# PCCproject/PCC-RL

Measured on AMD Instinct MI355X. Metric: env steps/sec (whole node) at 64k parallel envs, higher is better.
Workload: dtype f64; 1 GPU; BASELINE config 3: 65536 envs/GPU, 1 sender, per-env randomized bw/latency/queue/loss (ICML'19 ranges), U(-1,1) actions, 400-step episodes, auto-reset; envs_per_gpu=65536, senders=1, episode_return_allgathers=0, step_launches=two (send_kernel, retire_kernel)

## Files before the change

pcc-rl_amd/csrc/pcc_dev.h:

```cpp
#pragma once
#include <hip/hip_runtime.h>
#include <cstddef>

#include <cmath>
#include <cstdarg>
#include <cstdint>
#include <cstdio>
#include <cstdlib>
#include <cstring>
#include <atomic>
#include <new>
#include <vector>

#include "pcc_sim.h"

namespace pcc {

constexpr int kMaxFeatures = 16;
constexpr int kMaxSenders = 2;
constexpr int kWave = 64;
constexpr int kRetireBlock = 128;
#ifndef PCC_RETIRE_OCC
#define PCC_RETIRE_OCC 4
#endif
// ... 35 lines not shown
    uint32_t ha, hd, ta, td;
    uint32_t mi_sent;
    uint32_t ring_held[kMaxTiers];
    uint32_t cwnd;
    uint32_t heap_n;
    uint32_t send_cost;
    float ack_rate, loss_rate;
    uint32_t on_return_a, on_return_d;
};
static_assert(sizeof(EnvBlk) == 128 && sizeof(SndBlk) == 128, "one line per block");

struct NoiseOut {
    double now, q, tu, nsend;
    uint32_t sent, acked, lost, flags;
    uint32_t seq, pad[3];
};
static_assert(sizeof(NoiseOut) == 64, "one 64-byte record per env");

struct Dev {
    int64_t n;
    int ns, H, F, HF;
    int32_t fid[kMaxFeatures];
    int n_tiers;
    uint32_t cap0;
    char *tier_base[kMaxTiers];
    uint32_t *pool_free;
    size_t pool_free_stride;
    uint32_t *pool_share;
    int32_t *tier_top;
    uint32_t tier_slots[kMaxTiers];
    uint32_t parts, parts_shift, part_envs;
    uint32_t key0, key1, gid_base;
    uint32_t params_gen;
    double delta_scale;
    uint32_t max_steps;
    uint32_t *cls_count;
    uint32_t *cls_list;
    uint32_t *cursors;
    uint32_t *fctl;
    unsigned long long *q_entries;
    uint32_t q_cap;
    uint32_t fused_acquire;
    uint32_t fused_spin_ticks;
    uint32_t fused_debug;
    uint32_t fused_partial_naps;
    uint32_t fused_max_naps;
    uint32_t *any_done;
    uint32_t step_seq;
    uint64_t *timeline;
    unsigned long long *pass_stats;
    int pass_counters;
    uint32_t light_snake, wave_oldest_first, prio_level, prio_light_items, prio_wave_items, prio_team;
    uint32_t retire_sorted;
    int debug_skip;
    uint32_t round_packets, takeover_lanes, send_envs_per_wave, send_waves;
    double heavy_predict;
    double team_predict;
    float heavy_item_packets;
    float light_half_predict;
    float retire_wide_predict;
    double lo[5], hi[5];
    int rng_mode;
    const double *trace;
    int64_t trace_stride;
    const double *p_bw, *p_dl, *p_queue, *p_loss, *p_rate0;
    EnvBlk *env;
    SndBlk *snd;
    int64_t stride;
    char *shadow_rings;
    uint32_t *refill_count;
    uint32_t *refill_list;
    int shadows;
    unsigned long long *restart_stats;
    int use_cwnd;
    int use_noise;
    int engine;
    double noise_span;
    uint32_t noise_cap;
    double2 *noise_heap;
    double2 *noise_rtt;
    NoiseOut *noise_out;
    uint32_t noise_seq;
    float *hist;
    double2 *ring;
};

}
using namespace pcc;

namespace {

#ifndef PCC_PROFILE
#define PCC_PROFILE 0
#endif
constexpr bool kProfile = PCC_PROFILE != 0;
__device__ __forceinline__ bool prof_on(const Dev &D) { return kProfile && D.timeline != nullptr; }
__device__ __forceinline__ bool prof_counters(const Dev &D) { return kProfile && D.pass_counters != 0; }
__device__ __forceinline__ bool prof_skip(const Dev &D, int bit) { return kProfile && (D.debug_skip & bit) != 0; }

__device__ __forceinline__ double max0(double x) { return x > 0.0 ? x : 0.0; }

__device__ __forceinline__ void set_prio(uint32_t level) {
    if (level == 1u) __builtin_amdgcn_s_setprio(1);
    else if (level == 2u) __builtin_amdgcn_s_setprio(2);
    else if (level >= 3u) __builtin_amdgcn_s_setprio(3);
    else __builtin_amdgcn_s_setprio(0);
}

__device__ __forceinline__ uint64_t mul_wide_u32(uint32_t a, uint32_t b) {
    uint64_t r;
    asm("v_mad_u64_u32 %0, vcc, %1, %2, 0" : "=v"(r) : "v"(a), "v"(b) : "vcc");
    return r;
}

__device__ __forceinline__ void philox4x32_10(uint32_t c0, uint32_t c1, uint32_t c2, uint32_t c3, uint32_t k0,
                                              uint32_t k1, uint32_t (&out)[4]) {
#pragma unroll
    for (int r = 0; r < 10; r++) {
        const uint64_t p0 = mul_wide_u32(c0, 0xD2511F53u), p1 = mul_wide_u32(c2, 0xCD9E8D57u);
        const uint32_t hi0 = (uint32_t)(p0 >> 32), lo0 = (uint32_t)p0;
        const uint32_t hi1 = (uint32_t)(p1 >> 32), lo1 = (uint32_t)p1;
        const uint32_t n0 = hi1 ^ c1 ^ k0, n2 = hi0 ^ c3 ^ k1;
        c0 = n0; c1 = lo1; c2 = n2; c3 = lo0;
        k0 += 0x9E3779B9u; k1 += 0xBB67AE85u;
    }
    out[0] = c0; out[1] = c1; out[2] = c2; out[3] = c3;
}

__device__ __forceinline__ void philox4x32_10_sched(uint32_t c0, uint32_t c1, uint32_t c2, uint32_t c3, uint32_t k0,
                                                    uint32_t k1, uint32_t (&out)[4]) {
#pragma unroll
    for (int r = 0; r < 10; r++) {
        const uint64_t p0 = (uint64_t)c0 * 0xD2511F53u, p1 = (uint64_t)c2 * 0xCD9E8D57u;
        const uint32_t hi0 = (uint32_t)(p0 >> 32), lo0 = (uint32_t)p0;
        const uint32_t hi1 = (uint32_t)(p1 >> 32), lo1 = (uint32_t)p1;
        const uint32_t n0 = hi1 ^ c1 ^ k0, n2 = hi0 ^ c3 ^ k1;
        c0 = n0; c1 = lo1; c2 = n2; c3 = lo0;
        k0 += 0x9E3779B9u; k1 += 0xBB67AE85u;
    }
    out[0] = c0; out[1] = c1; out[2] = c2; out[3] = c3;
}

__device__ __forceinline__ double u32_to_unit(uint32_t x) { return (double)x * (1.0 / 4294967296.0); }

__device__ __forceinline__ double philox_packet_uniform(const Dev &D, uint32_t gid, uint32_t episode, uint32_t mi,
                                                        uint32_t j) {
    uint32_t w[4];
    philox4x32_10(j >> 2, mi, episode, gid, D.key0, D.key1, w);
    const uint32_t i = j & 3u;
    return u32_to_unit(i == 0 ? w[0] : i == 1 ? w[1] : i == 2 ? w[2] : w[3]);
}

__device__ __forceinline__ double2 link_send(double t, bool rnd , double dl,
                                             double maxq, double ebw, double &q, double &tu, bool &dropped) {
    const double qcur = max0(q - (t - tu));
    const double lat0 = dl + qcur;
    const bool full = ebw + qcur > maxq;
    const double grown = qcur + ebw;
    q = rnd ? q : (full ? qcur : grown);
    tu = rnd ? tu : t;
    dropped = rnd || full;
    double2 rec;
    rec.x = t + lat0;
    rec.y = lat0;
    return rec;
}

constexpr double kNearTol = 1e-12;
// ... 247 lines not shown
```

pcc-rl_amd/csrc/pcc_retire.hip:

```cpp
#include "pcc_retire_env.h"
#include "pcc_kernels.h"

#ifndef PCC_RETIRE_OCC2
#define PCC_RETIRE_OCC2 3
#endif

namespace {

constexpr int kRetireMaxPerBlock = kRetireBlock / 8;

__device__ __forceinline__ float *pol_lds() {
    extern __shared__ float s_pol_dyn[];
    return s_pol_dyn;
}

__device__ __forceinline__ const PolicyArgs &pol_arg(const PolicyArgs &p) { return p; }

template <int NS, bool NOISE, typename... Pol>
__global__ __launch_bounds__(kRetireBlock, NS == 2 ? PCC_RETIRE_OCC2 : PCC_RETIRE_OCC) void retire_kernel(Dev D, int read_buf, int fill_buf, int warm,
                                                              uint32_t warm_mi, int last_warm, int gate, int restart, float *obs_out,
                                                              float *reward_out, uint8_t *done_out, double *steps_out,
                                                              const void *actions, int actions_f64, Pol... pol) {
    constexpr bool POLICY = sizeof...(Pol) > 0;
    if (gate && __hip_atomic_load(D.any_done, __ATOMIC_RELAXED, __HIP_MEMORY_SCOPE_AGENT) != D.step_seq) return;
    __shared__ uint32_t s_env[kRetireMaxPerBlock], s_cls[kRetireMaxPerBlock], s_arrived;
    const uint32_t tid = threadIdx.x;
    if (prof_on(D) && !warm) {
        for (int64_t slot = (int64_t)blockIdx.x * kRetireBlock + tid; slot < 2 * D.n; slot += (int64_t)gridDim.x * kRetireBlock)
            D.timeline[slot * 8] = 0;
    }
    if (prof_on(D) && !warm && blockIdx.x < 8u && tid == 0 && D.n >= 1024)
        D.timeline[(int64_t)19 * D.n + 24 + blockIdx.x] = ((uint64_t)D.step_seq << 8) | xcc_id();
    const uint32_t lane = tid & (kWave - 1);
    if (tid == 0) s_arrived = 0u;
    if (tid < (uint32_t)kRetireMaxPerBlock) s_env[tid] = 0xFFFFFFFFu;
    if constexpr (POLICY) {
        float *w = pol_lds() + kRetireMaxPerBlock * kPolScratch;
        for (int k = (int)tid; k < pol_arg(pol...).n_params; k += kRetireBlock) w[k] = pol_arg(pol...).params[k];
    }
    __syncthreads();
    int64_t i = D.n;
    bool wide = false;
    const uint32_t P = D.parts, part = blockIdx.x % P, b_loc = blockIdx.x / P, grid_loc = gridDim.x / P;
    if (read_buf >= 0) {
        const uint32_t view = list_view(D, read_buf, part);
        const uint32_t row_mine = lane < (uint32_t)kClasses ? (uint32_t)(kClasses - 1) - lane : (uint32_t)kRestart;
        const uint32_t n_mine = lane <= (uint32_t)kClasses ? *cls_count_of(D, view, row_mine) : 0u;
        uint32_t incl = n_mine;
        for (int o = 1; o <= kClasses; o <<= 1) {
            const uint32_t up = (uint32_t)__shfl_up((int)incl, o);
            if (lane >= (uint32_t)o) incl += up;
        }
        const uint32_t total = rl_u32(incl, kClasses);
        const int cls_wide = NOISE ? kClasses : (D.retire_wide_predict >= 1e9f ? kClasses : class_of(D.retire_wide_predict));
        uint32_t n_top = cls_wide < kClasses ? rl_u32(incl, (uint32_t)(kClasses - 1 - cls_wide)) : 0u;
        {
            const uint32_t narrow_all = (total + 15u) / 16u;
            const uint32_t spare = grid_loc > narrow_all + 1u ? grid_loc - narrow_all - 1u : 0u;
            if (n_top > 16u * spare) n_top = 16u * spare;
        }
        const uint32_t wg_wide = (n_top + 7u) / 8u;
        wide = b_loc < wg_wide;
        uint32_t p;
        bool has;
        if (wide) {
            p = b_loc * 8u + tid / 16u;
            has = p < n_top;
        } else {
            p = n_top + (b_loc - wg_wide) * 16u + tid / 8u;
            has = p < total;
        }
        uint32_t lo_l = 0, hi_l = (uint32_t)kClasses;
        for (int it = 0; it < 6; it++) {
            const uint32_t mid = (lo_l + hi_l) >> 1;
            const uint32_t v = (uint32_t)__shfl((int)incl, (int)mid);
            if (lo_l < hi_l) { if (v > p) hi_l = mid; else lo_l = mid + 1u; }
        }
        const uint32_t L = lo_l;
        const uint32_t inc_L = (uint32_t)__shfl((int)incl, (int)L), n_L = (uint32_t)__shfl((int)n_mine, (int)L);
        if (has) {
            const uint32_t row = L < (uint32_t)kClasses ? (uint32_t)(kClasses - 1) - L : (uint32_t)kRestart;
            const uint32_t off = p - (inc_L - n_L);
            i = (int64_t)cls_list_of(D, view, row)[off];
        }
    } else {
        i = (int64_t)blockIdx.x * kRetireMaxPerBlock + tid / 8u;
    }
    float pred = -1.0f;
    Group g;
    uint32_t slot;
    bool glead;
    if (wide) {
        g.lane = tid & 15u;
        g.shift = lane & ~15u;
        slot = tid / 16u;
        glead = g.lane == 0;
        if (i < D.n) {
            pred = retire_env<NS, NOISE, 16>(D, i, g, warm, warm_mi, last_warm, restart, obs_out, reward_out, done_out, steps_out,
                                             actions, actions_f64);
            if constexpr (POLICY)
                policy_group<16>(pol_arg(pol...), pol_lds() + kRetireMaxPerBlock * kPolScratch, pol_lds() + slot * kPolScratch, obs_out + i * D.HF,
                                 i, D.n, g.lane, pol_arg(pol...).t0 + 1);
        }
    } else {
        g.lane = tid & 7u;
        g.shift = lane & ~7u;
        slot = tid / 8u;
        glead = g.lane == 0;
        if (i < D.n) {
            pred = retire_env<NS, NOISE, 8>(D, i, g, warm, warm_mi, last_warm, restart, obs_out, reward_out, done_out, steps_out,
                                            actions, actions_f64);
            if constexpr (POLICY)
                policy_group<8>(pol_arg(pol...), pol_lds() + kRetireMaxPerBlock * kPolScratch, pol_lds() + slot * kPolScratch, obs_out + i * D.HF,
                                i, D.n, g.lane, pol_arg(pol...).t0 + 1);
        }
    }
    if (fill_buf < 0) return;
    if (glead) {
        const bool restarted = pred == -2.0f;
        s_env[slot] = (pred != -1.0f) ? (uint32_t)i : 0xFFFFFFFFu;
        s_cls[slot] = restarted ? (uint32_t)kRestart : (uint32_t)class_of(pred);
    }
    __threadfence_block();
    uint32_t before = 0u;
    if (lane == 0) before = atomicAdd(&s_arrived, 1u);
    before = (uint32_t)__builtin_amdgcn_readfirstlane((int)before);
    if (before != kRetireBlock / kWave - 1) return;
    constexpr int kPerBlock = kRetireMaxPerBlock;
    const uint32_t e = lane < (uint32_t)kPerBlock ? s_env[lane & (kPerBlock - 1)] : 0xFFFFFFFFu;
    const uint32_t c = lane < (uint32_t)kPerBlock ? s_cls[lane & (kPerBlock - 1)] : 0xFFFFFFFFu;
// ... 42 lines not shown
```

pcc-rl_amd/csrc/pcc_retire_env.h:

```cpp
#pragma once
#include "pcc_dev.h"

namespace {

struct Group {
    uint32_t lane;
    uint32_t shift;
};

template <int G>
__device__ __forceinline__ uint32_t gballot(const Group &g, bool p) {
    return (uint32_t)(__ballot(p) >> g.shift) & ((1u << G) - 1u);
}

template <int G>
__device__ __forceinline__ double gbcast(double v, uint32_t src) { return __shfl(v, (int)src, G); }
template <int G>
__device__ __forceinline__ uint32_t gbcast(uint32_t v, uint32_t src) { return (uint32_t)__shfl((int)v, (int)src, G); }
template <int G>
__device__ __forceinline__ uint32_t gbcast(const Group &g, uint32_t v, uint32_t src) {
    return (uint32_t)__builtin_amdgcn_ds_bpermute((int)((g.shift + (src & (uint32_t)(G - 1))) << 2), (int)v);
}
template <int G>
__device__ __forceinline__ double gbcast(const Group &g, double v, uint32_t src) {
    const int idx = (int)((g.shift + (src & (uint32_t)(G - 1))) << 2);
    const int lo = __builtin_amdgcn_ds_bpermute(idx, __double2loint(v)), hi = __builtin_amdgcn_ds_bpermute(idx, __double2hiint(v));
    return __hiloint2double(hi, lo);
}

template <int G>
__device__ __forceinline__ uint32_t search_boundary(const Group &g, const double2 *ring, uint32_t mask, uint32_t lo,
                                                    uint32_t hi, double add, double end) {
    while (hi - lo > (uint32_t)G) {
        const uint32_t stride = (hi - lo + G - 1) / G;
        uint32_t sidx = lo + (g.lane + 1) * stride;
        if (sidx > hi) sidx = hi;
        sidx -= 1;
        const bool pass = ld_t1(ring + (sidx & mask)) + add < end;
        const uint32_t mfail = ~gballot<G>(g, pass) & ((1u << G) - 1u);
        if (!mfail) return hi;
        const uint32_t f = (uint32_t)__ffs((int)mfail) - 1u;
        const uint32_t s_f = gbcast<G>(g, sidx, f);
        if (f) lo = gbcast<G>(g, sidx, f - 1) + 1;
        hi = s_f;
        if (hi < lo) hi = lo;
    }
    const uint32_t k = lo + g.lane;
    const bool fail = k < hi && !(ld_t1(ring + (k & mask)) + add < end);
    const uint32_t m = gballot<G>(g, fail);
    return m ? lo + (uint32_t)__ffs((int)m) - 1u : hi;
}

struct Bound {
    uint32_t b;
    bool clean;
    double t, lat;
};

template <int K, int G>
__device__ __forceinline__ void search_many(const Group &g, const double2 *const (&ring)[K], const uint32_t (&mask)[K],
                                            const uint32_t (&lo0)[K], const uint32_t (&hi0)[K], const double (&add)[K],
                                            double end, const uint32_t (&hint)[K], Bound (&out)[K],
                                            unsigned long long *stat = nullptr ) {
    static_assert(K == 4 && (G == 16 || G == 8), "four searches per group of 16 or 8 lanes");
    constexpr int R = 16 / G;
    uint32_t lo[K], hi[K];
    bool inside[K], below[K];
    bool all_inside = true;
    auto window = [&](const bool (&need)[K], const bool last) {
        double2 r[K][R];
        uint32_t base[K];
#pragma unroll
        for (int k = 0; k < K; k++) {
            base[k] = lo[k] - lo0[k] >= 2u ? lo[k] - 2u : lo0[k];
#pragma unroll
            for (int h = 0; h < R; h++) {
                const uint32_t idx = base[k] + (uint32_t)(h * G) + g.lane;
                r[k][h].x = 0.0; r[k][h].y = 0.0;
                if (need[k] && idx < hi0[k]) r[k][h] = ld_rec(ring[k] + (idx & mask[k]));
            }
        }
#pragma unroll
        for (int k = 0; k < K; k++) {
            if (!need[k]) continue;
            uint32_t mpass = 0, m = 0, mnear = 0;
#pragma unroll
            for (int h = 0; h < R; h++) {
                const uint32_t idx = base[k] + (uint32_t)(h * G) + g.lane;
                const bool in = idx < hi0[k];
                const bool passes = in && (r[k][h].x + add[k] < end);
                mpass |= gballot<G>(g, passes) << (h * G);
                m |= gballot<G>(g, in && idx >= lo[k] && idx < hi[k] && !passes) << (h * G);
                double tn = gbcast<G>(g, r[k][h].x, (g.lane + 1u) & (uint32_t)(G - 1));
                if (h + 1 < R) {
                    const double tw = gbcast<G>(g, r[k][h + 1 < R ? h + 1 : h].x, 0u);
                    if (g.lane == (uint32_t)G - 1u) tn = tw;
                }
                const bool has_next = (h + 1 < R) || g.lane + 1 < (uint32_t)G;
                const bool nr = in && (idx + 1 < hi0[k]) && has_next && near_time(r[k][h].x, tn);
                mnear |= gballot<G>(g, nr) << (h * G);
            }
            const uint32_t b = m ? base[k] + (uint32_t)__ffs((int)m) - 1u : hi[k];
            const bool lo_ok = lo[k] == lo0[k] || ((mpass >> (lo[k] - 1u - base[k])) & 1u);
            const bool hi_ok = hi[k] == hi0[k] || !((mpass >> (hi[k] - base[k])) & 1u);
            inside[k] = last || (lo_ok && hi_ok);
            below[k] = !lo_ok;
            if (!inside[k]) {
                if (!lo_ok) { hi[k] = lo[k] - 1u; lo[k] = lo0[k]; }
                else { lo[k] = hi[k] + 1u; hi[k] = hi0[k]; }
                continue;
            }
            uint32_t want = 0;
            for (int d = 0; d < 3; d++) {
                const int l = (int)(b - base[k]) - 2 + d;
                if (l >= 0 && l < 16) want |= 1u << l;
            }
            out[k].b = b;
            out[k].clean = (mnear & want) == 0u;
            const uint32_t lb = b - base[k] < 16u ? b - base[k] : 0u;
            double bx = r[k][0].x, by = r[k][0].y;
            if (R > 1 && lb >= (uint32_t)G) { bx = r[k][R - 1].x; by = r[k][R - 1].y; }
            out[k].t = gbcast<G>(g, bx, lb & (G - 1));
            out[k].lat = gbcast<G>(g, by, lb & (G - 1));
        }
    };
    bool need[K];
#pragma unroll
    for (int k = 0; k < K; k++) {
        uint32_t h = hint[k] < lo0[k] ? lo0[k] : (hint[k] > hi0[k] ? hi0[k] : hint[k]);
        lo[k] = h - lo0[k] >= 5u ? h - 5u : lo0[k];
        hi[k] = hi0[k] - lo[k] > 12u ? lo[k] + 12u : hi0[k];
        need[k] = true;
    }
    window(need, false);
#pragma unroll
    for (int k = 0; k < K; k++) all_inside = all_inside && inside[k];
    if (kProfile && stat) {
        if (g.lane == 0) {
            atomicAdd(&stat[0], (unsigned long long)K);
            atomicAdd(&stat[1], (unsigned long long)((inside[0] ? 1 : 0) + (inside[1] ? 1 : 0) + (inside[2] ? 1 : 0) + (inside[3] ? 1 : 0)));
        }
        const uint64_t act = __ballot(true), hit = __ballot(all_inside);
        if ((threadIdx.x & (kWave - 1)) == (uint32_t)__ffsll((unsigned long long)act) - 1u) {
            atomicAdd(&stat[2], 1ull);
            if (act == hit) atomicAdd(&stat[3], 1ull);
        }
    }
    if (all_inside) return;
    constexpr int LQ = G / 4;
    constexpr int PL = 4 / LQ;
    const uint32_t q = g.lane / LQ, j = g.lane % LQ;
    uint32_t lo_m = q == 0 ? lo[0] : q == 1 ? lo[1] : q == 2 ? lo[2] : lo[3];
    uint32_t hi_m = q == 0 ? hi[0] : q == 1 ? hi[1] : q == 2 ? hi[2] : hi[3];
    const bool done_m = q == 0 ? inside[0] : q == 1 ? inside[1] : q == 2 ? inside[2] : inside[3];
    const double2 *ring_m = q == 0 ? ring[0] : q == 1 ? ring[1] : q == 2 ? ring[2] : ring[3];
    const uint32_t mask_m = q == 0 ? mask[0] : q == 1 ? mask[1] : q == 2 ? mask[2] : mask[3];
    const double add_m = q == 0 ? add[0] : q == 1 ? add[1] : q == 2 ? add[2] : add[3];
    const bool below_m = q == 0 ? below[0] : q == 1 ? below[1] : q == 2 ? below[2] : below[3];
    bool first = true;
    for (;;) {
        const bool active = !done_m && hi_m - lo_m > 12u;
        if (!gballot<G>(g, active)) break;
        const uint32_t stride = (hi_m - lo_m + 3u) / 4u;
        uint32_t sidx[PL];
        uint32_t passbits = 0;
#pragma unroll
        for (int e = 0; e < PL; e++) {
            const uint32_t pr = j * PL + (uint32_t)e;
            uint32_t x = lo_m + (pr + 1u) * stride;
            if (x > hi_m) x = hi_m;
            if (first) {
                if (below_m) {
                    const uint32_t dist = 12u << (2u * (3u - pr));
                    x = hi_m - lo_m > dist ? hi_m - dist + 1u : lo_m + 1u;
                } else {
                    const uint32_t dist = 12u << (2u * pr);
                    x = hi_m - lo_m > dist ? lo_m + dist : hi_m;
                }
            }
            sidx[e] = x - 1u;
        }
        first = false;
        double tsamp[PL];
#pragma unroll
        for (int e = 0; e < PL; e++) {
            tsamp[e] = 0.0;
            if (active) tsamp[e] = ld_t1(ring_m + (sidx[e] & mask_m));
        }
#pragma unroll
        for (int e = 0; e < PL; e++) {
            const uint32_t bm = gballot<G>(g, tsamp[e] + add_m < end) >> (LQ * q);
#pragma unroll
            for (int l = 0; l < LQ; l++) passbits |= ((bm >> l) & 1u) << (l * PL + e);
        }
        const uint32_t mfail = ~passbits & 0xFu;
        const uint32_t f = mfail ? (uint32_t)__ffs((int)mfail) - 1u : 0u;
        const uint32_t fp = f ? f - 1u : 0u;
        uint32_t mine_f = sidx[0], mine_p = sidx[0];
        if (PL > 1) { mine_f = (f % PL) ? sidx[PL - 1] : sidx[0]; mine_p = (fp % PL) ? sidx[PL - 1] : sidx[0]; }
        const uint32_t s_f = gbcast<G>(g, mine_f, LQ * q + f / PL);
        const uint32_t s_p = gbcast<G>(g, mine_p, LQ * q + fp / PL);
        const uint32_t s_last = gbcast<G>(g, sidx[PL - 1], LQ * q + LQ - 1);
        if (active) {
            if (!mfail) {
                lo_m = s_last + 1u;
            } else {
                if (f) lo_m = s_p + 1u;
                hi_m = s_f < lo_m ? lo_m : s_f;
            }
        }
    }
#pragma unroll
    for (int k = 0; k < K; k++) {
        need[k] = !inside[k];
        if (need[k]) { lo[k] = gbcast<G>(g, lo_m, LQ * k); hi[k] = gbcast<G>(g, hi_m, LQ * k); }
    }
    window(need, true);
}


__device__ __forceinline__ void rotate_to_front(double2 *ring, uint32_t mask, uint32_t p, uint32_t k) {
    const double2 r = ld_rec(ring + (k & mask));
    for (uint32_t m = k; m > p; m--) st_rec(ring + (m & mask), ld_rec(ring + ((m - 1) & mask)));
    st_rec(ring + (p & mask), r);
}

struct DropFix { uint32_t p, cand_idx; double cand_t, cand_lat; };
struct Cand { double t, lat; };

template <int G>
__device__ __forceinline__ void near_window_g(const Group &g, const double2 *ring, uint32_t mask, uint32_t h, uint32_t tail,
                                              uint32_t b, uint32_t &g0, uint32_t &g1) {
    g0 = b;
    g1 = b;
    if (b > h) {
        g0 = b - 1;
        for (;;) {
            const bool has = g0 - h >= g.lane;
            const double t = has ? ld_t1(ring + ((g0 - g.lane) & mask)) : 0.0;
            const double tp = gbcast<G>(g, t, (g.lane + 1u) & (uint32_t)(G - 1));
            const bool nr = g.lane + 1u < (uint32_t)G && g0 - h >= g.lane + 1u && near_time(tp, t);
            const uint32_t run = (uint32_t)__ffs((int)~gballot<G>(g, nr)) - 1u;
            g0 -= run;
            if (run < (uint32_t)G - 1u) break;
        }
    }
    if (b < tail) {
        g1 = b + 1;
        for (;;) {
            const bool has = g1 - 1u + g.lane < tail;
            const double t = has ? ld_t1(ring + ((g1 - 1u + g.lane) & mask)) : 0.0;
            const double tn = gbcast<G>(g, t, (g.lane + 1u) & (uint32_t)(G - 1));
            const bool nr = g.lane + 1u < (uint32_t)G && g1 + g.lane < tail && near_time(tn, t);
            const uint32_t run = (uint32_t)__ffs((int)~gballot<G>(g, nr)) - 1u;
            g1 += run;
            if (run < (uint32_t)G - 1u) break;
        }
    }
}

__device__ __forceinline__ DropFix fix_drop_window(double2 *ring, uint32_t mask, uint32_t g0, uint32_t g1, double dl, double end) {
    uint32_t p = g0;
    for (uint32_t k = g0; k < g1; k++) {
        const double2 r = ld_rec(ring + (k & mask));
        if (r.x + dl < end) {
            if (k != p) rotate_to_front(ring, mask, p, k);
            p++;
        }
    }
    DropFix out;
    out.p = p; out.cand_idx = 0xFFFFFFFFu; out.cand_t = INFINITY; out.cand_lat = 0.0;
    for (uint32_t k = p; k < g1; k++) {
        const double2 r = ld_rec(ring + (k & mask));
        if (r.x < end) {
            const double t2 = r.x + dl, l2 = r.y + dl;
            if (out.cand_idx == 0xFFFFFFFFu || t2 < out.cand_t || (t2 == out.cand_t && l2 < out.cand_lat)) {
                out.cand_idx = k; out.cand_t = t2; out.cand_lat = l2;
            }
        }
    }
    return out;
}

template <int G>
__device__ __forceinline__ void gmin_key(double &t, double &lat, uint32_t &idx) {
#pragma unroll
    for (int o = G / 2; o >= 1; o >>= 1) {
        const double ot = __shfl_xor(t, o, G), ol = __shfl_xor(lat, o, G);
        const uint32_t oi = (uint32_t)__shfl_xor((int)idx, o, G);
        const bool take = oi != 0xFFFFFFFFu && (idx == 0xFFFFFFFFu || ot < t || (ot == t && (ol < lat || (ol == lat && oi < idx))));
        if (take) { t = ot; lat = ol; idx = oi; }
// ... 489 lines not shown
        }
    }
#pragma unroll
    for (int s = 0; s < NS; s++) {
        D.snd[sidx(D, s, i)].heap_n = hn[s];
        o.nsend[s] = nsend[s];
    }
    D.env[i].ep_draws = ep_draws;
    D.env[i].mi_draws = mi_draws;
    o.now = now; o.q = q; o.tu = tu;
    return o;
}

template <int NS>
__device__ __forceinline__ void release_ring_slots(const Dev &D, const int64_t i, const bool push = true) {
#pragma unroll
    for (int s = 0; s < NS; s++) {
        const int64_t k = sidx(D, s, i);
        for (int c = 1; c < D.n_tiers; c++) {
            const uint32_t held = D.snd[k].ring_held[c];
            if (held) {
                if (push) pool_push(D, (uint32_t)c, held - 1u);
                D.snd[k].ring_held[c] = 0;
            }
        }
        D.snd[k].ring_tier = 0;
        D.snd[k].ring_base = D.tier_base[0] + (size_t)((int64_t)i * NS + s) * tier_slot_bytes(D, 0);
    }
}

template <int NS>
__device__ __forceinline__ void reset_env(const Dev &D, const int64_t i, float *obs_out) {
    const uint32_t episode = D.env[i].episode;
    D.env[i].episode = episode + 1;

    double bw, lat, queue, loss, rate0[NS];
    const int64_t ie = env_of(D, i);
    if (D.p_bw) {
        bw = D.p_bw[ie]; lat = D.p_dl[ie]; queue = D.p_queue[ie]; loss = D.p_loss[ie];
#pragma unroll
        for (int s = 0; s < NS; s++) rate0[s] = D.p_rate0[(int64_t)s * D.n + ie];
    } else {
        uint32_t w0[4], w1[4];
        const uint32_t gid = D.gid_base + (uint32_t)ie;
        philox4x32_10(0u, kParamTag, episode, gid, D.key0, D.key1, w0);
        philox4x32_10(1u, kParamTag, episode, gid, D.key0, D.key1, w1);
        bw = D.lo[0] + (D.hi[0] - D.lo[0]) * u32_to_unit(w0[0]);
        lat = D.lo[1] + (D.hi[1] - D.lo[1]) * u32_to_unit(w0[1]);
        queue = (double)(1 + (long long)exp(D.lo[2] + (D.hi[2] - D.lo[2]) * u32_to_unit(w0[2])));
        loss = D.lo[3] + (D.hi[3] - D.lo[3]) * u32_to_unit(w0[3]);
#pragma unroll
        for (int s = 0; s < NS; s++) rate0[s] = (D.lo[4] + (D.hi[4] - D.lo[4]) * u32_to_unit(w1[s])) * bw;
    }
    bool bad = !(bw > 0.0) || !(bw <= 1e8) || !(lat > 0.0) || !(lat <= 1e6) || !(queue >= 1.0) || !(queue <= 1e9) ||
               !(loss >= 0.0) || !(loss <= 1.0);
#pragma unroll
    for (int s = 0; s < NS; s++) bad = bad || !(rate0[s] > 0.0) || !(rate0[s] <= 1e9);
    if (bad) {
        D.env[i].flags |= PCC_FLAG_BAD_PARAMS;
        bw = 100.0; lat = 0.1; queue = 2.0; loss = 0.0;
#pragma unroll
        for (int s = 0; s < NS; s++) rate0[s] = 100.0;
    }
    D.env[i].bw = bw; D.env[i].dl = lat; D.env[i].lr = loss;
    D.env[i].maxq = queue / bw;
    D.env[i].ebw = 1.0 / bw;
    D.env[i].q = 0.0; D.env[i].tu = 0.0; D.env[i].now = 0.0;
    D.env[i].run_dur = 3 * lat;
    D.env[i].steps = 0;
    D.env[i].done = 0;
    D.env[i].mi_draws = 0; D.env[i].ep_draws = 0;
#pragma unroll
    for (int s = 0; s < NS; s++) {
        const int64_t k = sidx(D, s, i);
        D.snd[k].rate = rate0[s];
        D.snd[k].rate0 = rate0[s];
        D.snd[k].next_send = 1.0 / rate0[s];
        D.snd[k].ha = 0; D.snd[k].hd = 0; D.snd[k].ta = 0; D.snd[k].td = 0; D.snd[k].mi_sent = 0;
        D.snd[k].cwnd = 25;
        D.snd[k].heap_n = 0;
        D.snd[k].min_lat = 0.0;
        D.snd[k].ack_rate = 0.f; D.snd[k].loss_rate = 0.f; D.snd[k].on_return_a = 0; D.snd[k].on_return_d = 0;
        D.snd[k].ep_return = 0.0;
        float *hist = D.hist + ((int64_t)ie * NS + s) * D.HF;
        float *obs = obs_out ? obs_out + ((int64_t)ie * NS + s) * D.HF : nullptr;
        for (int h = 0; i < D.n && h < D.H; h++)
            for (int f = 0; f < D.F; f++) {
                const int id = D.fid[f];
                const double v = (id == PCC_M_SEND_RATIO || id == PCC_M_LATENCY_RATIO) ? 1.0 : 0.0;
                const float x = (float)(v / c_metric_scale[id]);
                hist[h * D.F + f] = x;
                if (obs) obs[h * D.F + f] = x;
            }
    }
}

template <int NS, bool NOISE, int G>
__device__ __forceinline__ float retire_env(const Dev &D, const int64_t i, const Group g, int warm, uint32_t warm_mi,
                                            int last_warm, int restart, float *obs_out, float *reward_out, uint8_t *done_out,
                                            double *steps_out, const void *actions, int actions_f64) {
    if (warm && !D.env[i].resetting) return -1.0f;
    const bool lead = g.lane == 0;
    const bool tl = prof_on(D) && (threadIdx.x & (kWave - 1)) == 0;
    uint64_t *tlw = prof_on(D) ? D.timeline + (int64_t)2 * D.n * 8 + (int64_t)blockIdx.x * 16 : nullptr;
    uint64_t tl_t = tl ? wall_clock64() : 0;
    if (tl && threadIdx.x == 0) tlw[0] = tl_t;
#define PCC_TL_STAMP(slot)                                                                               \
    if (tl) {                                                                                            \
        const uint64_t t_now = wall_clock64();                                                           \
        atomicAdd(reinterpret_cast<unsigned long long *>(&tlw[slot]), (unsigned long long)(t_now - tl_t)); \
        tl_t = t_now;                                                                                    \
    }

    const double dl = D.env[i].dl;
    const double start = D.env[i].now;
    const double run_dur = D.env[i].run_dur;
    const double end = start + run_dur;
    const uint32_t steps = D.env[i].steps;
    const unsigned long long total_before = D.env[i].total_sent;
    double now = start;

    double nsend[NS];
    uint32_t ha[NS], hd[NS], ta[NS], td[NS], sent[NS], acked[NS], lost[NS], from[NS];
    double2 *ra[NS], *rd[NS];
    uint32_t amask[NS], dmasks[NS];
#pragma unroll
    for (int s = 0; s < NS; s++) {
        const int64_t k = sidx(D, s, i);
        nsend[s] = D.snd[k].next_send;
        ha[s] = D.snd[k].ha; hd[s] = D.snd[k].hd; ta[s] = D.snd[k].ta; td[s] = D.snd[k].td;
        sent[s] = D.snd[k].mi_sent;
        acked[s] = lost[s] = 0;
        from[s] = ha[s];
        const RingRef rr = ring_ref(D, k);
        ra[s] = rr.accepted(); rd[s] = rr.dropped();
        amask[s] = rr.mask(); dmasks[s] = rr.dmask();
    }
    uint32_t flags = 0;
    double noise_rate[NS];
#pragma unroll
    for (int s = 0; s < NS; s++) noise_rate[s] = 0.0;

    if constexpr (NOISE) {
        double rate[NS];
        uint32_t cw[NS];
#pragma unroll
        for (int s = 0; s < NS; s++) {
            const int64_t k = sidx(D, s, i);
            rate[s] = D.snd[k].rate;
            cw[s] = D.use_cwnd ? D.snd[k].cwnd : 0xFFFFFFFFu;
            if (!warm) {
                const int64_t ar = D.use_cwnd ? 2 * (i * NS + s) : i * NS + s;
                double delta = actions_f64 ? ((const double *)actions)[ar] : (double)((const float *)actions)[ar];
                if (delta != delta) { delta = 0.0; flags |= PCC_FLAG_BAD_ACTION; }
                delta *= D.delta_scale;
                rate[s] = delta >= 0.0 ? rate[s] * (1.0 + delta) : rate[s] / (1.0 - delta);
                if (rate[s] > kMaxRate) rate[s] = kMaxRate;
                if (rate[s] < kMinRate) rate[s] = kMinRate;
                if (D.use_cwnd) {
                    double dc = actions_f64 ? ((const double *)actions)[ar + 1] : (double)((const float *)actions)[ar + 1];
                    if (dc != dc) { dc = 0.0; flags |= PCC_FLAG_BAD_ACTION; }
                    dc *= D.delta_scale;
                    const double c = dc >= 0.0 ? (double)cw[s] * (1.0 + dc) : (double)cw[s] / (1.0 - dc);
                    cw[s] = c >= 5000.0 ? 5000u : (c < 4.0 ? 4u : (uint32_t)c);
                    if (lead) D.snd[k].cwnd = cw[s];
                }
            }
// ... 128 lines not shown
                    uint64_t pos = 0;
#pragma unroll
                    for (int x = 0; x < NS; x++) pos += (uint64_t)ta[x] + td[x];
                    if ((int64_t)pos >= D.trace_stride) { flags |= PCC_FLAG_TRACE_OVERRUN; u = 1.0; }
                    else u = D.trace[i * D.trace_stride + pos];
                } else {
                    uint32_t j = 0;
#pragma unroll
                    for (int x = 0; x < NS; x++) j += sent[x];
                    if (D.use_cwnd) j = D.env[i].mi_draws;
                    u = philox_packet_uniform(D, D.gid_base + (uint32_t)env_of(D, i), D.env[i].episode - 1,
                                              warm ? warm_mi : steps + 2, j);
                }
                if (D.use_cwnd && D.rng_mode == PCC_RNG_TRACE) {
                    const uint32_t pos = D.env[i].ep_draws;
                    if ((int64_t)pos >= D.trace_stride) { flags |= PCC_FLAG_TRACE_OVERRUN; u = 1.0; }
                    else u = D.trace[i * D.trace_stride + pos];
                }
                const bool can_send = !D.use_cwnd || (ta[s] - ha[s]) + (td[s] - hd[s]) < D.snd[sidx(D, s, i)].cwnd;
                if (D.use_cwnd && lead) D.env[i].ep_draws += 1u;
                const double rate = D.snd[sidx(D, s, i)].rate;
                sent[s] += can_send ? 1u : 0u;
                nsend[s] = t + 1.0 / rate;
                bool dropped;
                const double2 rec = link_send(t, u < D.env[i].lr, dl, D.env[i].maxq, D.env[i].ebw, q, tu, dropped);
                if (!can_send) {
                } else if (dropped) {
                    if (lead) st_rec(rd[s] + (td[s] & dmasks[s]), rec);
                    td[s]++;
                } else {
                    if (lead) st_rec(ra[s] + (ta[s] & amask[s]), rec);
                    ta[s]++;
                }
                if (ta[s] - ha[s] > amask[s] + 1u || td[s] - hd[s] > dmasks[s] + 1u) flags |= PCC_FLAG_RING_OVERFLOW;
                if (lead) { D.env[i].q = q; D.env[i].tu = tu; }
            }
        }
        (void)l_h2;
    }

    PCC_TL_STAMP(6)
    unsigned long long sent_total = 0;
#pragma unroll
    for (int s = 0; s < NS; s++) sent_total += sent[s];
    if (now * (64.0 * kNearTol) > D.env[i].ebw) flags |= PCC_FLAG_TIME_RANGE;
    if (lead) {
        if (flags) D.env[i].flags |= flags;
#pragma unroll
        for (int s = 0; s < NS; s++) {
            const int64_t k = sidx(D, s, i);
            D.snd[k].ha = ha[s]; D.snd[k].hd = hd[s]; D.snd[k].ta = ta[s]; D.snd[k].td = td[s];
        }
    }
    if (warm) {
        if (lead) {
            D.env[i].now = now;
            D.env[i].total_sent = total_before + sent_total;
#pragma unroll
            for (int s = 0; s < NS; s++) D.snd[sidx(D, s, i)].next_send = nsend[s];
            if (last_warm) D.env[i].resetting = 0;
        }
        return -1.0f;
    }

    bool need_halves = steps_out != nullptr;
    for (int f = 0; f < D.F; f++) {
        const int id = D.fid[f];
        need_halves |= (id == PCC_M_LATENCY_INCREASE || id == PCC_M_ACK_LATENCY_INFLATION ||
                        id == PCC_M_SENT_LATENCY_INFLATION);
    }
    const double dur = now - start;
    double new_run_dur = run_dur, rate_sum = 0.0;
    uint32_t cost_word = 0, sent_all = 0;
#pragma unroll
    for (int s = 0; s < NS; s++) sent_all += sent[s];
#pragma unroll
    for (int s = 0; s < NS; s++) {
        const int64_t k = sidx(D, s, i);
        double lat = 0.0, inc = 0.0;
        PCC_TL_STAMP(7)
        if (acked[s] > 0 && !prof_skip(D, 1))
            rtt_means<G>(g, ra[s], amask[s], from[s], acked[s], NOISE ? 0.0 : dl, need_halves, lat, inc);
        PCC_TL_STAMP(8)
        float *hist = D.hist + ((int64_t)i * NS + s) * D.HF;
        const int keep = D.HF - D.F;
        constexpr int kRows = 32 / G;
        const bool small_hist = D.HF <= kRows * G;
        float old_row[kRows];
#pragma unroll
        for (int b = 0; b < kRows; b++) old_row[b] = 0.f;
        if (small_hist) {
#pragma unroll
            for (int b = 0; b < kRows; b++) {
                const int x = b * G + (int)g.lane;
                if (x < keep) old_row[b] = hist[x + D.F];
            }
        }
        double min_lat = D.snd[k].min_lat;
        if (s == 0) cost_word = D.snd[k].send_cost;
        const double ep_before = D.snd[k].ep_return;
        const double rate_now = NOISE ? noise_rate[s] : D.snd[k].rate;
        rate_sum += rate_now;
        double m[PCC_N_METRICS];
        mi_metrics(sent[s], acked[s], lost[s], dur, lat, inc, min_lat, m);
        PCC_TL_STAMP(9)
        const double reward =
            (10.0 * m[PCC_M_RECV_RATE] / (double)(8 * kBytesPerPacket) - 1e3 * m[PCC_M_AVG_LATENCY] -
             2e3 * m[PCC_M_LOSS_RATIO]) * kRewardScale;
        if (s == 0 && m[PCC_M_AVG_LATENCY] > 0.0) new_run_dur = 0.5 * m[PCC_M_AVG_LATENCY];

        float *obs = obs_out ? obs_out + ((int64_t)i * NS + s) * D.HF : nullptr;
        float nf0 = 0.f, nf1 = 0.f;
        for (int f = 0; f < D.F; f++) {
            const int id = D.fid[f];
            double val;
            switch (id) {
                case 0: val = m[0] / 1e7; break;
                case 1: val = m[1] / 1e7; break;
                case 2: val = m[2]; break;
                case 3: val = m[3]; break;
                case 4: val = m[4]; break;
                case 5: val = m[5]; break;
                case 6: val = m[6]; break;
                case 7: val = m[7]; break;
                case 8: val = m[8]; break;
                case 9: val = m[9]; break;
                case 10: val = m[10]; break;
                default: val = m[11]; break;
            }
            static_assert(PCC_M_SEND_RATE == 0 && PCC_M_RECV_RATE == 1 && PCC_N_METRICS == 12, "the switch above");
            if (((keep + f) & (G - 1)) == (int)g.lane) { if (f < G) nf0 = (float)val; else nf1 = (float)val; }
        }
        const bool restarts = restart && steps + 1 >= D.max_steps;
        if (small_hist) {
#pragma unroll
            for (int b = 0; b < kRows; b++) {
                const int x = b * G + (int)g.lane;
                float v = (x - keep) < G ? nf0 : nf1;
                if (x < keep) v = old_row[b];
                if (x < D.HF && !prof_skip(D, 2)) {
                    if (restarts) {
                        const int id = D.fid[x % D.F];
                        v = (float)(((id == PCC_M_SEND_RATIO || id == PCC_M_LATENCY_RATIO) ? 1.0 : 0.0) / c_metric_scale[id]);
                    }
                    hist[x] = v;
                    if (obs) obs[x] = v;
                }
            }
        } else {
            for (int base = 0; base < D.HF && !prof_skip(D, 2); base += G) {
                const int x = base + (int)g.lane;
                float v = (x - keep) < G ? nf0 : nf1;
                if (x < keep) v = hist[x + D.F];
                if (x < D.HF) {
                    if (restarts) {
                        const int id = D.fid[x % D.F];
                        v = (float)(((id == PCC_M_SEND_RATIO || id == PCC_M_LATENCY_RATIO) ? 1.0 : 0.0) / c_metric_scale[id]);
                    }
                    hist[x] = v;
                    if (obs) obs[x] = v;
                }
            }
        }
        PCC_TL_STAMP(10)
        if (lead) {
            const double ret = ep_before + reward;
            D.snd[k].next_send = nsend[s]; D.snd[k].min_lat = min_lat;
// ... 89 lines not shown
```

pcc-rl_amd/csrc/pcc_sim.hip:

```cpp
#include <functional>

#include "pcc_kernels.h"
#include "pcc_policy.h"

using namespace pcc;

namespace {

const double h_metric_min[PCC_N_METRICS] = {0.0, 0.0, 0.0, 0.0, 0.0, 0.0, -1.0, -1.0, 0.0, 0.0, 1.0, 0.0};
const double h_metric_max[PCC_N_METRICS] = {1e9, 1e9, 100.0, 100.0, 100.0, 1.0, 10.0, 10.0, 100.0, 100.0, 10000.0, 1000.0};
const double h_metric_scale[PCC_N_METRICS] = {1e7, 1e7, 1.0, 1.0, 1.0, 1.0, 1.0, 1.0, 1.0, 1.0, 1.0, 1.0};

thread_local char g_err[512] = "";

int fail(int code, const char *fmt, ...) {
    va_list ap;
    va_start(ap, fmt);
    vsnprintf(g_err, sizeof g_err, fmt, ap);
    va_end(ap);
    return code;
}

}

// ... 18 lines not shown
    void *list_blob;
    size_t list_bytes;
    void *noise_blob;
    void *noise_out_blob;
    uint32_t light_front;
    int noise_sorted;
    size_t noise_bytes;
    uint32_t ring_capacity;
    bool pools_pending;
    bool restarts_pending;
    bool read_has_restarts;
    uint32_t list_min_envs;
    hipStream_t aux_wave, aux_restart;
    hipEvent_t ev_fork, ev_wave;
    double retire_grid_frac;
    uint32_t step_seq;
    void *shadow_blob;
    size_t shadow_bytes;
    hipEvent_t ev_ret, ev_refill[4];
    bool refill_recorded[4];
    hipStream_t last_stream;
    int fused;
    int xcc_count;
    int clean_buf;
    int fused_blocks[2];
    uint32_t fused_light_wgs;
    uint32_t fused_light_front;
    unsigned long long fused_steps;
    int rollout_epilogue;
    float *roll_act;
    size_t roll_act_floats;
};

namespace {

struct DeviceGuard {
    int prev = -1;
    bool switched = false;
    explicit DeviceGuard(int dev) {
        if (hipGetDevice(&prev) == hipSuccess && prev != dev) switched = hipSetDevice(dev) == hipSuccess;
    }
    ~DeviceGuard() {
        if (switched) (void)hipSetDevice(prev);
    }
};

std::vector<hipStream_t *> side_streams(pcc_sim *sim) { return {&sim->aux_wave, &sim->aux_restart}; }
std::vector<hipEvent_t *> events(pcc_sim *sim) {
    return {&sim->ev_fork, &sim->ev_wave, &sim->ev_ret, &sim->ev_refill[0], &sim->ev_refill[1], &sim->ev_refill[2], &sim->ev_refill[3]};
}

struct Carver {
    char *base;
    size_t off = 0;
    explicit Carver(char *b) : base(b) {}
    template <typename T>
    T *take(size_t count) {
        off = (off + 255) & ~(size_t)255;
        T *p = base ? reinterpret_cast<T *>(base + off) : nullptr;
        off += count * sizeof(T);
        return p;
    }
};

size_t carve_state(Dev &d, char *base) {
    Carver c(base);
    const size_t n = (size_t)d.n, sn = n * d.ns;
    d.env = c.take<EnvBlk>(2 * n);
    d.snd = c.take<SndBlk>(2 * sn);
    d.stride = (int64_t)(2 * n);
    d.refill_count = c.take<uint32_t>(4 * kCntStride);
    d.refill_list = c.take<uint32_t>(4 * n);
    d.restart_stats = c.take<unsigned long long>(2);
    d.cls_count = c.take<uint32_t>(kListBufs * kParts * kClsStride);
    d.cursors = c.take<uint32_t>(kListBufs * kParts * kShards * kCursorStride);
    d.fctl = c.take<uint32_t>(kListBufs * kXcds * kFctlWords * kCursorStride);
    d.q_cap = n <= ((size_t)1 << 22) ? (uint32_t)n : 0u;
    d.q_entries = c.take<unsigned long long>((size_t)2 * kXcds * d.q_cap);
    d.any_done = c.take<uint32_t>(1);
    d.tier_top = c.take<int32_t>(kMaxTiers * kParts * kTopStride);
    d.pool_share = c.take<uint32_t>(kMaxTiers);
    d.pool_free_stride = sn < 256 ? 256 : sn;
    d.pool_free = c.take<uint32_t>(kMaxTiers * d.pool_free_stride);
    d.hist = c.take<float>(sn * d.HF);
    return (c.off + 255) & ~(size_t)255;
}

int check_hip(hipError_t err, const char *what) {
    if (err == hipSuccess) return PCC_OK;
    return fail(PCC_EHIP, "%s: %s", what, hipGetErrorString(err));
}

bool uses_lists(const pcc_sim_t *sim) { return sim->d.n >= (int64_t)sim->list_min_envs; }

struct StepOut { float *obs, *reward; uint8_t *done; double *steps; };

StepOut row_of(const Dev &d, const StepOut &o, int t) {
    const size_t row = (size_t)d.n * d.ns, k = (size_t)t;
    return {o.obs ? o.obs + k * row * d.HF : nullptr, o.reward ? o.reward + k * row : nullptr, o.done ? o.done + k * (size_t)d.n : nullptr,
            o.steps ? o.steps + k * row * PCC_STEP_COLS : nullptr};
}

int64_t wave_path_wgs(const pcc_sim_t *sim) {
    const Dev &d = sim->d;
    const int64_t P = d.parts;
    int64_t waves = (int64_t)sim->cu_count * d.send_waves;
    if (waves > d.n) waves = d.n;
    return P * (((waves + 3) / 4 + P - 1) / P);
}

unsigned few_envs_grid(const pcc_sim_t *sim) {
    const int64_t wgs = (sim->d.n + 3) / 4;
    return (unsigned)(sim->cu_count < wgs ? sim->cu_count : wgs);
}

int launch_send(pcc_sim_t *sim, int warm, uint32_t warm_mi, int gate, const void *actions, int actions_f64, hipStream_t st) {
    const Dev &d = sim->d;
    const bool tr = d.rng_mode == PCC_RNG_TRACE;
    const bool lists = uses_lists(sim);
    const int read_buf = (warm || !lists) ? -1 : sim->read_buf;
    const int zero_buf = lists ? sim->fill_buf : -1;
    const bool rs = read_buf >= 0 && sim->read_has_restarts;
    const int64_t E = d.send_envs_per_wave, P = d.parts;
    unsigned light_grid = (unsigned)(((d.n + E - 1) / E + 3) / 4), wave_grid = 0u, front = 0u;
    if (read_buf >= 0) {
        const int64_t E_min = d.light_half_predict < 1e9f && E >= 2 ? E / 2 : E;
        const int64_t light_items_part = ((int64_t)d.part_envs + E_min - 1) / E_min + kClasses;
        light_grid = (unsigned)(P * ((light_items_part + 3) / 4));
        const bool wave = !d.use_cwnd && d.heavy_predict < 1e9;
        if (wave) wave_grid = (unsigned)wave_path_wgs(sim);
        if (wave && !rs) front = (unsigned)((int64_t)sim->light_front * P);
        if (front > light_grid) front = light_grid / (unsigned)P * (unsigned)P;
    }
    auto main_launch = [&](hipStream_t s) {
        pcc::launch_send(d, tr, light_grid, wave_grid, front, s, read_buf, zero_buf, warm, warm_mi, gate, actions, actions_f64);
    };
    if (!rs) {
        main_launch(st);
    } else if (d.shadows) {
        const unsigned restart_grid = few_envs_grid(sim);
        main_launch(st);
        launch_send_restart(d, tr, restart_grid < 32u ? restart_grid : 32u, st, read_buf, actions, actions_f64);
    } else {
        if (hipEventRecord(sim->ev_fork, st) != hipSuccess) return fail(PCC_EHIP, "hipEventRecord failed");
        (void)hipStreamWaitEvent(sim->aux_wave, sim->ev_fork, 0);
        main_launch(sim->aux_wave);
        (void)hipEventRecord(sim->ev_wave, sim->aux_wave);
        launch_send_restart(d, tr, few_envs_grid(sim), st, read_buf, actions, actions_f64);
        (void)hipStreamWaitEvent(st, sim->ev_wave, 0);
    }
    if (rs && !warm) sim->restarts_pending = false;
    return check_hip(hipGetLastError(), "send kernel launch");
}

int launch_retire_half(pcc_sim_t *sim, int warm, uint32_t warm_mi, int last_warm, int gate, int restart, const StepOut &out,
                       hipStream_t st, const PolicyArgs *pol = nullptr) {
    const Dev &d = sim->d;
    const bool lists = uses_lists(sim);
    const int read = (warm || !d.retire_sorted || !lists) ? -1 : sim->read_buf;
    const int64_t narrow = (d.n + kRetireEnvsPerBlockNarrow - 1) / kRetireEnvsPerBlockNarrow;
    const int64_t narrow_part = ((int64_t)d.part_envs + kRetireEnvsPerBlockNarrow - 1) / kRetireEnvsPerBlockNarrow;
    const unsigned grid = (unsigned)(read >= 0 ? (int64_t)d.parts * (narrow_part + (int64_t)(sim->retire_grid_frac * (double)narrow_part) + 1) : narrow);
    const int fill = (warm || !lists) ? -1 : sim->fill_buf;
    launch_retire(d, false, grid, st, read, fill, warm, warm_mi, last_warm, gate, restart, out.obs, out.reward, out.done, out.steps,
                  nullptr, 0, pol);
    const int rc = check_hip(hipGetLastError(), "retire kernel launch");
    if (rc == PCC_OK && !warm && lists) {
// ... 993 lines not shown
```

Baseline: 405.5 million env steps/s.

## Add optional hist padding, scalar class-count loads, and aligned ring windows

Three compile-time experiments, all off by default. The first pads each per-sender history row to a 32-float line. The second loads the class counts through the scalar constant address space in an unrolled loop. The third aligns the ring search windows to multiples of 8 and adds an optional second narrowing pass. Window comparisons are rewritten to wrap-safe signed range checks, and the hist pointer now uses a stride field, so these changes alter the default path a little even with every flag at zero.

```diff
diff --git a/pcc-rl_amd/csrc/pcc_dev.h b/pcc-rl_amd/csrc/pcc_dev.h
--- a/pcc-rl_amd/csrc/pcc_dev.h
+++ b/pcc-rl_amd/csrc/pcc_dev.h
@@ -141,8 +141,14 @@
     NoiseOut *noise_out;
     uint32_t noise_seq;
     float *hist;
+    int hist_stride;
     double2 *ring;
 };
+
+#ifndef PCC_HIST_LINE
+#define PCC_HIST_LINE 0
+#endif
+inline int hist_stride_for(int HF) { return (PCC_HIST_LINE && HF <= 32) ? 32 : HF; }
 
 }
 using namespace pcc;
diff --git a/pcc-rl_amd/csrc/pcc_retire.hip b/pcc-rl_amd/csrc/pcc_retire.hip
--- a/pcc-rl_amd/csrc/pcc_retire.hip
+++ b/pcc-rl_amd/csrc/pcc_retire.hip
@@ -1,6 +1,9 @@
 #include "pcc_retire_env.h"
 #include "pcc_kernels.h"
 
+#ifndef PCC_CNT_SCALAR
+#define PCC_CNT_SCALAR 0
+#endif
 #ifndef PCC_RETIRE_OCC2
 #define PCC_RETIRE_OCC2 3
 #endif
@@ -45,7 +48,22 @@
     if (read_buf >= 0) {
         const uint32_t view = list_view(D, read_buf, part);
         const uint32_t row_mine = lane < (uint32_t)kClasses ? (uint32_t)(kClasses - 1) - lane : (uint32_t)kRestart;
+#if PCC_CNT_SCALAR
+        uint32_t n_mine = 0u;
+        {
+            const __attribute__((address_space(4))) uint32_t *cnt =
+                (const __attribute__((address_space(4))) uint32_t *)(const void *)cls_count_of(D, view, 0u);
+#pragma unroll
+            for (uint32_t l = 0; l <= (uint32_t)kClasses; l++) {
+                const uint32_t row = l < (uint32_t)kClasses ? (uint32_t)(kClasses - 1) - l : (uint32_t)kRestart;
+                const uint32_t v = cnt[(size_t)row * kCntStride];
+                if (lane == l) n_mine = v;
+            }
+        }
+        (void)row_mine;
+#else
         const uint32_t n_mine = lane <= (uint32_t)kClasses ? *cls_count_of(D, view, row_mine) : 0u;
+#endif
         uint32_t incl = n_mine;
         for (int o = 1; o <= kClasses; o <<= 1) {
             const uint32_t up = (uint32_t)__shfl_up((int)incl, o);
diff --git a/pcc-rl_amd/csrc/pcc_retire_env.h b/pcc-rl_amd/csrc/pcc_retire_env.h
--- a/pcc-rl_amd/csrc/pcc_retire_env.h
+++ b/pcc-rl_amd/csrc/pcc_retire_env.h
@@ -51,6 +51,10 @@
     return m ? lo + (uint32_t)__ffs((int)m) - 1u : hi;
 }
 
+#ifndef PCC_WIN_ALIGN
+#define PCC_WIN_ALIGN 0
+#endif
+#define PCC_BETWEEN(i, a, b) ((int32_t)((i) - (a)) >= 0 && (int32_t)((i) - (b)) < 0)
 struct Bound {
     uint32_t b;
     bool clean;
@@ -66,18 +70,30 @@
     constexpr int R = 16 / G;
     uint32_t lo[K], hi[K];
     bool inside[K], below[K];
+    auto base_of = [&](const int k, const bool last) -> uint32_t {
+#if PCC_WIN_ALIGN
+        if (last) {
+            const uint32_t al = (lo[k] - 2u) & ~7u;
+            return hi[k] + 1u - al < 16u ? al : lo[k] - 2u;
+        }
+        return (lo[k] == lo0[k] ? lo[k] : lo[k] - 2u) & ~7u;
+#else
+        (void)last;
+        return lo[k] - lo0[k] >= 2u ? lo[k] - 2u : lo0[k];
+#endif
+    };
     bool all_inside = true;
     auto window = [&](const bool (&need)[K], const bool last) {
         double2 r[K][R];
         uint32_t base[K];
 #pragma unroll
         for (int k = 0; k < K; k++) {
-            base[k] = lo[k] - lo0[k] >= 2u ? lo[k] - 2u : lo0[k];
+            base[k] = base_of(k, last);
 #pragma unroll
             for (int h = 0; h < R; h++) {
                 const uint32_t idx = base[k] + (uint32_t)(h * G) + g.lane;
                 r[k][h].x = 0.0; r[k][h].y = 0.0;
-                if (need[k] && idx < hi0[k]) r[k][h] = ld_rec(ring[k] + (idx & mask[k]));
+                if (need[k] && PCC_BETWEEN(idx, lo0[k], hi0[k])) r[k][h] = ld_rec(ring[k] + (idx & mask[k]));
             }
         }
 #pragma unroll
@@ -87,22 +103,22 @@
 #pragma unroll
             for (int h = 0; h < R; h++) {
                 const uint32_t idx = base[k] + (uint32_t)(h * G) + g.lane;
-                const bool in = idx < hi0[k];
+                const bool in = PCC_BETWEEN(idx, lo0[k], hi0[k]);
                 const bool passes = in && (r[k][h].x + add[k] < end);
                 mpass |= gballot<G>(g, passes) << (h * G);
-                m |= gballot<G>(g, in && idx >= lo[k] && idx < hi[k] && !passes) << (h * G);
+                m |= gballot<G>(g, in && PCC_BETWEEN(idx, lo[k], hi[k]) && !passes) << (h * G);
                 double tn = gbcast<G>(g, r[k][h].x, (g.lane + 1u) & (uint32_t)(G - 1));
                 if (h + 1 < R) {
                     const double tw = gbcast<G>(g, r[k][h + 1 < R ? h + 1 : h].x, 0u);
                     if (g.lane == (uint32_t)G - 1u) tn = tw;
                 }
                 const bool has_next = (h + 1 < R) || g.lane + 1 < (uint32_t)G;
-                const bool nr = in && (idx + 1 < hi0[k]) && has_next && near_time(r[k][h].x, tn);
+                const bool nr = in && (int32_t)(idx + 1u - hi0[k]) < 0 && has_next && near_time(r[k][h].x, tn);
                 mnear |= gballot<G>(g, nr) << (h * G);
             }
             const uint32_t b = m ? base[k] + (uint32_t)__ffs((int)m) - 1u : hi[k];
-            const bool lo_ok = lo[k] == lo0[k] || ((mpass >> (lo[k] - 1u - base[k])) & 1u);
-            const bool hi_ok = hi[k] == hi0[k] || !((mpass >> (hi[k] - base[k])) & 1u);
+            const bool lo_ok = lo[k] == lo0[k] || ((mpass >> ((lo[k] - 1u - base[k]) & 31u)) & 1u);
+            const bool hi_ok = hi[k] == hi0[k] || !((mpass >> ((hi[k] - base[k]) & 31u)) & 1u);
             inside[k] = last || (lo_ok && hi_ok);
             below[k] = !lo_ok;
             if (!inside[k]) {
@@ -127,9 +143,19 @@
     bool need[K];
 #pragma unroll
     for (int k = 0; k < K; k++) {
-        uint32_t h = hint[k] < lo0[k] ? lo0[k] : (hint[k] > hi0[k] ? hi0[k] : hint[k]);
-        lo[k] = h - lo0[k] >= 5u ? h - 5u : lo0[k];
+        const uint32_t n = hi0[k] - lo0[k];
+        uint32_t hr = hint[k] - lo0[k];
+        if (hr > n) hr = (int32_t)hr < 0 ? 0u : n;
+        const uint32_t h = lo0[k] + hr;
+#if PCC_WIN_ALIGN
+        const uint32_t b0 = (h - 4u) & ~7u;
+        lo[k] = (int32_t)(b0 + 2u - lo0[k]) > 0 ? b0 + 2u : lo0[k];
+        const uint32_t top = base_of(k, false) + 14u;
+        hi[k] = top - lo0[k] < n ? top : hi0[k];
+#else
+        lo[k] = hr >= 5u ? h - 5u : lo0[k];
         hi[k] = hi0[k] - lo[k] > 12u ? lo[k] + 12u : hi0[k];
+#endif
         need[k] = true;
     }
     window(need, false);
@@ -147,6 +173,23 @@
         }
     }
     if (all_inside) return;
+#if PCC_WIN_ALIGN >= 2
+#pragma unroll
+    for (int k = 0; k < K; k++) {
+        need[k] = !inside[k];
+        if (!need[k]) continue;
+        if (below[k]) {
+            lo[k] = (int32_t)(hi[k] - 7u - lo0[k]) > 0 ? hi[k] - 7u : lo0[k];
+        } else {
+            hi[k] = lo[k] + 7u - lo0[k] < hi0[k] - lo0[k] ? lo[k] + 7u : hi0[k];
+        }
+    }
+    window(need, false);
+    all_inside = true;
+#pragma unroll
+    for (int k = 0; k < K; k++) all_inside = all_inside && inside[k];
+    if (all_inside) return;
+#endif
     constexpr int LQ = G / 4;
     constexpr int PL = 4 / LQ;
     const uint32_t q = g.lane / LQ, j = g.lane % LQ;
@@ -168,7 +211,7 @@
         for (int e = 0; e < PL; e++) {
             const uint32_t pr = j * PL + (uint32_t)e;
             uint32_t x = lo_m + (pr + 1u) * stride;
-            if (x > hi_m) x = hi_m;
+            if (x - lo_m > hi_m - lo_m) x = hi_m;
             if (first) {
                 if (below_m) {
                     const uint32_t dist = 12u << (2u * (3u - pr));
@@ -206,7 +249,7 @@
                 lo_m = s_last + 1u;
             } else {
                 if (f) lo_m = s_p + 1u;
-                hi_m = s_f < lo_m ? lo_m : s_f;
+                hi_m = (int32_t)(s_f - lo_m) < 0 ? lo_m : s_f;
             }
         }
     }
@@ -862,7 +905,7 @@
         D.snd[k].min_lat = 0.0;
         D.snd[k].ack_rate = 0.f; D.snd[k].loss_rate = 0.f; D.snd[k].on_return_a = 0; D.snd[k].on_return_d = 0;
         D.snd[k].ep_return = 0.0;
-        float *hist = D.hist + ((int64_t)ie * NS + s) * D.HF;
+        float *hist = D.hist + ((int64_t)ie * NS + s) * D.hist_stride;
         float *obs = obs_out ? obs_out + ((int64_t)ie * NS + s) * D.HF : nullptr;
         for (int h = 0; i < D.n && h < D.H; h++)
             for (int f = 0; f < D.F; f++) {
@@ -1157,7 +1200,7 @@
         if (acked[s] > 0 && !prof_skip(D, 1))
             rtt_means<G>(g, ra[s], amask[s], from[s], acked[s], NOISE ? 0.0 : dl, need_halves, lat, inc);
         PCC_TL_STAMP(8)
-        float *hist = D.hist + ((int64_t)i * NS + s) * D.HF;
+        float *hist = D.hist + ((int64_t)i * NS + s) * D.hist_stride;
         const int keep = D.HF - D.F;
         constexpr int kRows = 32 / G;
         const bool small_hist = D.HF <= kRows * G;
diff --git a/pcc-rl_amd/csrc/pcc_sim.hip b/pcc-rl_amd/csrc/pcc_sim.hip
--- a/pcc-rl_amd/csrc/pcc_sim.hip
+++ b/pcc-rl_amd/csrc/pcc_sim.hip
@@ -124,7 +124,8 @@
     d.pool_share = c.take<uint32_t>(kMaxTiers);
     d.pool_free_stride = sn < 256 ? 256 : sn;
     d.pool_free = c.take<uint32_t>(kMaxTiers * d.pool_free_stride);
-    d.hist = c.take<float>(sn * d.HF);
+    d.hist_stride = hist_stride_for(d.HF);
+    d.hist = c.take<float>(sn * (size_t)d.hist_stride);
     return (c.off + 255) & ~(size_t)255;
 }
 
```

After: 397.1 million env steps/s. 2.1% lower.
